# Kitware/SMQTK-Indexing

Hardware: AMD Instinct MI355X
Metric: queries/sec, exact brute-force l2 kNN k=100 over 10000000x128 float32 (recall@100 = 1.0 by construction); scan HBM GB/s vs 8 TB/s peak (higher is better)
Workload: dtype f32 results (distances bit-identical to numpy float32); filter arithmetic int8 MFMA (i32 accumulation, measured per-row error bound), exact re-rank f32

## Files before the change

### smqtk_indexing_amd/csrc/sq_dense_i8.hpp

```cpp
#pragma once
#include "sq_dense_scan.hpp"

namespace sq {

typedef int i32x4 __attribute__((ext_vector_type(4)));
typedef int i32x16 __attribute__((ext_vector_type(16)));

template <int KS>
struct I8Geom {
    static constexpr int ROW_BYTES = KS * 32;
    static constexpr int UNIT_ROWS = KS == 4 ? 64 : 32;
    static constexpr int TILES = UNIT_ROWS / 32;
    static constexpr int UNIT_BYTES = UNIT_ROWS * ROW_BYTES;
    static constexpr int SLOT_BYTES = UNIT_BYTES + 256;
    static constexpr int WAVES = KS <= 8 ? 8 : 4;
    static constexpr int NSTAGE = 2;
    static constexpr int PIECES = UNIT_BYTES / 1024;
    static constexpr int SAMPLES_PER_UNIT = 2 * TILES;
};
static constexpr int I8_MAX_ROW_BYTES = 512;
__host__ __device__ constexpr int i8_row_bytes(int d) { return d <= 128 ? 128 : (d <= 256 ? 256 : 512); }
__host__ __device__ constexpr int i8_unit_rows(int row_bytes) { return row_bytes == 128 ? 64 : 32; }

__device__ __forceinline__ float i8_element(float v, const float* __restrict__ center, int k, bool cosine, double inv_norm) {
    if (cosine) return (float)((double)v * inv_norm);
    return center ? __fsub_rn(v, center[k]) : v;
}

template <int EPL>
static __global__ __launch_bounds__(256) void dense8_energy_kernel(const float* __restrict__ db, long long n, long long ld, int d,
                                                                    const float* __restrict__ center, const double* __restrict__ nx64,
                                                                    double cap, double* __restrict__ sum) {
    __shared__ double red[4][2];
    const int lane = threadIdx.x & 63;
    const long long wave0 = (long long)blockIdx.x * 4 + (threadIdx.x >> 6), nw = (long long)gridDim.x * 4;
    double acc = 0.0, rows = 0.0;
    for (long long row = wave0; row < n; row += nw) {
        double e = 0.0;
        bool bad = false;
        const double inv_norm = nx64 ? 1.0 / sqrt(nx64[row]) : 1.0;
        for (int k0 = 0; k0 < d; k0 += 64 * EPL) {
#pragma unroll
            for (int j = 0; j < EPL; ++j) {
                const int k = k0 + EPL * lane + j;
                if (k < d) {
                    const float v = db[row * ld + k];
                    const float xc = i8_element(v, center, k, nx64 != nullptr, inv_norm);
                    if (!(fabsf(xc) < 3.0e38f)) bad = true;
                    e += (double)xc * (double)xc;
                }
            }
        }
        if (__ballot(bad) != 0ull) continue;
        for (int o = 32; o > 0; o >>= 1) e += __shfl_xor(e, o);
        if (e <= cap) {
            acc += e;
            rows += 1.0;
        }
    }
    if (lane == 0) {
        red[threadIdx.x >> 6][0] = acc;
        red[threadIdx.x >> 6][1] = rows;
    }
    __syncthreads();
    if (threadIdx.x == 0) {
        atomicAdd(sum, red[0][0] + red[1][0] + red[2][0] + red[3][0]);
        atomicAdd(sum + 1, red[0][1] + red[1][1] + red[2][1] + red[3][1]);
    }
}

static constexpr int I8_NCLIP = 12, I8_NCUT = 10;
struct Dense8ClipArgs {
    float inv_dx[I8_NCLIP], dx[I8_NCLIP];
    float cut[I8_NCLIP][I8_NCUT];
};

template <int EPL>
static __global__ __launch_bounds__(256) void dense8_clip_stats_kernel(const float* __restrict__ db, long long n, long long ld, int d,
                                                                        const float* __restrict__ center, const double* __restrict__ nx64,
                                                                        Dense8ClipArgs ca, u32* __restrict__ counts, int row_step) {
    const int lane = threadIdx.x & 63;
    const long long wave0 = ((long long)blockIdx.x * 4 + (threadIdx.x >> 6)) * row_step, nw = (long long)gridDim.x * 4 * row_step;
    u32 cnt[I8_NCLIP][I8_NCUT];
#pragma unroll
    for (int c = 0; c < I8_NCLIP; ++c)
#pragma unroll
        for (int m = 0; m < I8_NCUT; ++m) cnt[c][m] = 0u;
    for (long long row = wave0; row < n; row += nw) {
        float r2[I8_NCLIP];
#pragma unroll
        for (int c = 0; c < I8_NCLIP; ++c) r2[c] = 0.f;
        bool bad = false;
        const double inv_norm = nx64 ? 1.0 / sqrt(nx64[row]) : 1.0;
        for (int k0 = 0; k0 < d; k0 += 64 * EPL) {
#pragma unroll
            for (int j = 0; j < EPL; ++j) {
                const int k = k0 + EPL * lane + j;
                if (k < d) {
                    const float v = db[row * ld + k];
                    const float xc = i8_element(v, center, k, nx64 != nullptr, inv_norm);
                    if (!(fabsf(xc) < 3.0e38f)) bad = true;
#pragma unroll
                    for (int c = 0; c < I8_NCLIP; ++c) {
                        const float t = fminf(fmaxf(rintf(xc * ca.inv_dx[c]), -127.f), 127.f);
                        const float res = __fmaf_rn(-t, ca.dx[c], xc);
                        r2[c] = __fmaf_rn(res, res, r2[c]);
                    }
                }
            }
        }
        if (__ballot(bad) != 0ull) continue;
#pragma unroll
        for (int c = 0; c < I8_NCLIP; ++c) {
            for (int o = 32; o > 0; o >>= 1) r2[c] += __shfl_xor(r2[c], o);
#pragma unroll
            for (int m = 0; m < I8_NCUT; ++m) cnt[c][m] += r2[c] > ca.cut[c][m] ? 1u : 0u;
        }
    }
    if (lane == 0) {
#pragma unroll
        for (int c = 0; c < I8_NCLIP; ++c)
#pragma unroll
            for (int m = 0; m < I8_NCUT; ++m)
                if (cnt[c][m]) atomicAdd(&counts[c * I8_NCUT + m], cnt[c][m]);
    }
}

template <int EPL>
static __global__ __launch_bounds__(256) void dense8_build_kernel(const float* __restrict__ db, long long n, long long ld, int d,
                                                                   long long n_pad, const float* __restrict__ center,
                                                                   const double* __restrict__ nx64, float inv_dx, float dx,
                                                                   signed char* __restrict__ out8, float* __restrict__ nrow,
                                                                   float* __restrict__ r2row, long long row_base, int row_bytes) {
    const int lane = threadIdx.x & 63;
    const long long row = row_base + (long long)blockIdx.x * 4 + (threadIdx.x >> 6);
    if (row >= n_pad) return;
    double e2 = 0.0, r2 = 0.0;
    bool finite = true;
    const double inv_norm = (row < n && nx64) ? 1.0 / sqrt(nx64[row]) : 1.0;
    for (int k0 = 0; k0 < row_bytes; k0 += 64 * EPL) {
        unsigned char q[EPL];
#pragma unroll
        for (int j = 0; j < EPL; ++j) q[j] = 0;
        if (row < n) {
#pragma unroll
            for (int j = 0; j < EPL; ++j) {
                const int k = k0 + EPL * lane + j;
                if (k < d) {
                    const float v = db[row * ld + k];
                    const float xc = i8_element(v, center, k, nx64 != nullptr, inv_norm);
                    if (!(xc == xc) || !(fabsf(xc) < 3.0e38f)) finite = false;
                    float t = rintf(xc * inv_dx);
                    t = fminf(fmaxf(t, -127.f), 127.f);
                    if (!(t == t)) t = 0.f;
                    q[j] = (unsigned char)(signed char)(int)t;
                    const double res = (double)xc - (double)t * (double)dx;
                    e2 += (double)xc * (double)xc;
                    r2 += res * res;
                }
            }
        }
        if (k0 + EPL * lane >= row_bytes) continue;
        unsigned char* dst = reinterpret_cast<unsigned char*>(out8) + row * row_bytes + k0 + EPL * lane;
        if constexpr (EPL == 2) {
            *reinterpret_cast<unsigned short*>(dst) = (unsigned short)(q[0] | (q[1] << 8));
        } else if constexpr (EPL == 4) {
            *reinterpret_cast<u32*>(dst) = (u32)q[0] | ((u32)q[1] << 8) | ((u32)q[2] << 16) | ((u32)q[3] << 24);
        } else {
            uint2 w;
            w.x = (u32)q[0] | ((u32)q[1] << 8) | ((u32)q[2] << 16) | ((u32)q[3] << 24);
            w.y = (u32)q[4] | ((u32)q[5] << 8) | ((u32)q[6] << 16) | ((u32)q[7] << 24);
            *reinterpret_cast<uint2*>(dst) = w;
        }
    }
    finite = __ballot(!finite) == 0ull;
    for (int o = 32; o > 0; o >>= 1) {
        e2 += __shfl_xor(e2, o);
        r2 += __shfl_xor(r2, o);
    }
    if (lane == 0) {
        float nr = __builtin_inff(), rr = 0.f;
        if (row < n && finite) {
            nr = nx64 ? 0.f : (float)e2;
            if ((double)nr > e2) nr = __uint_as_float(__float_as_uint(nr) - 1u);
            rr = (float)r2;
            if ((double)rr < r2) rr = __uint_as_float(__float_as_uint(rr) + 1u);
        }
        nrow[row] = nr;
        r2row[row] = rr;
    }
}

static __global__ __launch_bounds__(256) void dense8_resid_stats_kernel(const float* __restrict__ r2row, const float* __restrict__ nrow,
                                                                         long long n, double* __restrict__ sum_r2,
                                                                         u32* __restrict__ max_bits) {
    __shared__ double red[4];
    __shared__ float rmax[4], nmax[4];
    double acc = 0.0;
    float m = 0.f, mn = 0.f;
    for (long long i = (long long)blockIdx.x * 256 + threadIdx.x; i < n; i += (long long)gridDim.x * 256) {
        const float nv = nrow[i];
        if (nv < __builtin_inff() && nv > -__builtin_inff()) {
            const float v = r2row[i];
            acc += (double)v;
            m = fmaxf(m, v);
            mn = fmaxf(mn, nv);
        }
    }
    for (int o = 32; o > 0; o >>= 1) {
        acc += __shfl_xor(acc, o);
        m = fmaxf(m, __shfl_xor(m, o));
        mn = fmaxf(mn, __shfl_xor(mn, o));
    }
    if ((threadIdx.x & 63) == 0) {
        red[threadIdx.x >> 6] = acc;
        rmax[threadIdx.x >> 6] = m;
        nmax[threadIdx.x >> 6] = mn;
    }
    __syncthreads();
    if (threadIdx.x == 0) {
        atomicAdd(sum_r2, red[0] + red[1] + red[2] + red[3]);
        atomicMax(max_bits, __float_as_uint(fmaxf(fmaxf(rmax[0], rmax[1]), fmaxf(rmax[2], rmax[3]))));
        atomicMax(max_bits + 1, __float_as_uint(fmaxf(fmaxf(nmax[0], nmax[1]), fmaxf(nmax[2], nmax[3]))));
    }
}

static __global__ __launch_bounds__(256) void dense8_flag_kernel(const float* __restrict__ r2row, float* __restrict__ nrow, long long n,
                                                                  float r2_cut, u32* __restrict__ flagged, long long row_base) {
    const long long i = row_base + (long long)blockIdx.x * 256 + threadIdx.x;
    if (i >= n) return;
    if (nrow[i] < __builtin_inff() && r2row[i] > r2_cut) {
        nrow[i] = -__builtin_inff();
        atomicAdd(flagged, 1u);
    }
}

template <int EPL>
__device__ __forceinline__ void dense8_prep_query_row(const float* __restrict__ qrow, bool real, int d, const float* __restrict__ center,
                                                      double dx, double r_max, double x_max, int cosine,
                                                      signed char* __restrict__ p0, signed char* __restrict__ p1, float2& par_out,
                                                      double& qn2_out) {
    const int l16 = threadIdx.x & 15;
    const float sc = cosine ? -1.f : -2.f;
    float v[EPL][4];
#pragma unroll
    for (int c = 0; c < EPL; ++c)
#pragma unroll
        for (int e = 0; e < 4; ++e) {
            const int t = 64 * c + l16 + 16 * e;
            float raw = 0.f, cen = 0.f;
            if (real && t < d) {
                raw = qrow[t];
                if (center) cen = center[t];
            }
            v[c][e] = (real && t < d) ? (center ? __fsub_rn(raw, cen) : raw) : 0.f;
        }
    auto chunk_sum = [](double x0, double x1, double x2, double x3) __attribute__((always_inline)) {
        double sacc = (x0 + x2) + (x1 + x3);
        for (int o = 8; o > 0; o >>= 1) sacc += __shfl_xor(sacc, o);
        return sacc;
    };
    if (cosine) {
        double nn = 0.0;
#pragma unroll
        for (int c = 0; c < EPL; ++c)
            nn += chunk_sum((double)v[c][0] * (double)v[c][0], (double)v[c][1] * (double)v[c][1], (double)v[c][2] * (double)v[c][2],
                            (double)v[c][3] * (double)v[c][3]);
        const double rn = sqrt(nn);
#pragma unroll
        for (int c = 0; c < EPL; ++c)
#pragma unroll
            for (int e = 0; e < 4; ++e) v[c][e] = (float)((double)v[c][e] / rn);
    }
    double Q = 0.0;
    float mx = 0.f;
#pragma unroll
    for (int c = 0; c < EPL; ++c) {
        Q += chunk_sum((double)v[c][0] * (double)v[c][0], (double)v[c][1] * (double)v[c][1], (double)v[c][2] * (double)v[c][2],
                       (double)v[c][3] * (double)v[c][3]);
#pragma unroll
        for (int e = 0; e < 4; ++e) {
            float m = fabsf(sc * v[c][e]);
            if (!(m == m)) m = __builtin_inff();
            mx = fmaxf(mx, m);
        }
    }
    for (int o = 8; o > 0; o >>= 1) mx = fmaxf(mx, __shfl_xor(mx, o));
    const bool ok = real && mx < 3.0e38f && mx > 0.f;
    const double dq = ok ? (double)mx / 127.0 : 1.0;
    const double inv_dq = 1.0 / dq;
    double r2s = 0.0;
#pragma unroll
    for (int c = 0; c < EPL; ++c) {
        double r2[4];
#pragma unroll
        for (int e = 0; e < 4; ++e) {
            const double w = (double)(sc * v[c][e]);
            const double ws = w * inv_dq;
            float qt8 = 0.f, ql8 = 0.f;
            if (ok) {
                qt8 = fminf(fmaxf(rintf((float)ws), -127.f), 127.f);
                ql8 = fminf(fmaxf(rintf((float)((ws - (double)qt8) * 256.0)), -127.f), 127.f);
            }
            const int t = 64 * c + l16 + 16 * e;
            p0[t] = (signed char)(int)qt8;
            p1[t] = (signed char)(int)ql8;
            const double res = w - ((double)qt8 + (double)ql8 * 0.00390625) * dq;
            r2[e] = res * res;
        }
        r2s += chunk_sum(r2[0], r2[1], r2[2], r2[3]);
    }
    const double rq = sqrt(r2s) * (1.0 + 1e-9);
    const double unit = dx * dq;
    const double xr = x_max + r_max, qn = sqrt(Q), wn = (cosine ? 1.0 : 2.0) * qn;
    double e = r_max * wn + xr * rq + 4.0 * 5.9604644775390625e-08 * (xr * (wn + rq) + x_max * x_max);
    e *= 1.0 + 1e-6;
    float ef = (float)e;
    if ((double)ef < e) ef = __uint_as_float(__float_as_uint(ef) + 1u);
    if (!ok && real) ef = __builtin_inff();
    par_out = make_float2((float)unit, real ? ef : 0.f);
    qn2_out = real ? Q : 0.0;
}

template <int EPL>
static __global__ __launch_bounds__(64) void dense8_prep_queries_kernel(const float* __restrict__ q, int nq, int d,
                                                                         const float* __restrict__ center, double dx, double r_max,
                                                                         double x_max, signed char* __restrict__ qs8,
                                                                         float2* __restrict__ par, double* __restrict__ qn2,
                                                                         float* __restrict__ thr, u32* __restrict__ cnt,
                                                                         u32* __restrict__ oflag, float* __restrict__ q_al, int ldq,
                                                                         const DenseCallPtrs* __restrict__ ind, int cosine, int plane_rows) {
    constexpr int row_bytes = EPL * 64;
    if (ind) q = ind->q;
    const int qi = blockIdx.x * 4 + (threadIdx.x >> 4), t = threadIdx.x & 15;
    if (t == 0) {
        thr[qi] = qi < nq ? -__builtin_inff() : __builtin_nanf("");
        cnt[qi] = 0u;
        if (qi == 0) *oflag = 0u;
    }
    if (qi < nq)
        for (int i = t; i < ldq; i += 16) q_al[(long long)qi * ldq + i] = i < d ? q[(long long)qi * d + i] : 0.f;
    float2 pr;
    double Q;
    dense8_prep_query_row<EPL>(q + (long long)qi * d, qi < nq, d, center, dx, r_max, x_max, cosine,
                               qs8 + (long long)qi * row_bytes, qs8 + (long long)(plane_rows + qi) * row_bytes, pr, Q);
    if (t == 0) {
        par[qi] = pr;
        qn2[qi] = Q;
    }
}

struct Dense8ThrPost {
    const float2* par;
    const double* qn2;
    __device__ __forceinline__ void prologue(int, double*) const {}
    __device__ __forceinline__ float operator()(int q, float t) const {
        if (!(t < __builtin_inff())) return t;
        if (!(par[q].y < __builtin_inff())) return __builtin_nanf("");
        const double tt = (double)t + 2.0 * (double)par[q].y + 4e-6 * fabs((double)t + qn2[q]);
        float r = (float)tt;
        if ((double)r < tt) r = __uint_as_float(__float_as_uint(r) + (r >= 0.f ? 1 : -1));
        return r;
    }
};

struct Dense8ScanArgs {
    const signed char* scan8;
    const float* nrow;
    long long n;
    long long n_units;
    const signed char* qs8;
    const float2* par;
    const float* thr;
    uint2* wave_out;
    u32* wave_cnt;
    u32 wave_cap;
    float* sample_out;
    long long ns;
    long long unit_step;
    long long n_sel;
    int nrb;
    int nt;
    long long nt_from_row;
    int nqt;
    int plane_rows;
    int debug;
    float* wave_score;
    u32* hist;
};

template <int KS>
__device__ __forceinline__ int i8_swz(int c, int r) {
    if constexpr (KS == 4) return c ^ ((r >> 1) & 7);
    return (c & ~15) | ((c & 15) ^ (r & 15));
}

enum { I8_EMIT = 0, I8_SAMPLE = 1, I8_LANEMIN = 2, I8_EMIT_H = 3 };

static constexpr int I8_HIST_BINS = 64;
static constexpr int I8_CNT_SHIFT = 5;
static constexpr int I8_HIST_WORDS = TILE_ROWS * I8_HIST_BINS + (TILE_ROWS << I8_CNT_SHIFT);

template <int WAVES>
__device__ __forceinline__ void dense8_hist_flush(u32* lds_hist, u32* __restrict__ ghist) {
    constexpr int PER = TILE_ROWS * I8_HIST_BINS / WAVES;
    const int lane = threadIdx.x & 63;
    const int wave = __builtin_amdgcn_readfirstlane(threadIdx.x >> 6);
#pragma unroll
    for (int i = 0; i < PER / 64; ++i) {
        const int b = wave * PER + i * 64 + lane;
        const u32 v = __hip_atomic_exchange(lds_hist + b, 0u, __ATOMIC_RELAXED, __HIP_MEMORY_SCOPE_WORKGROUP);
        if (v) __hip_atomic_fetch_add(ghist + b, v, __ATOMIC_RELAXED, __HIP_MEMORY_SCOPE_AGENT);
    }
}

template <int KS, int MODE>
__device__ __forceinline__ void dense8_stream(const Dense8ScanArgs& a, unsigned char* smem, const i32x4 (&bq)[KS], const i32x4 (&bl)[KS],
                                              float unit_lo, float thr_l, u32& wcount, float& smin, u32* lds_ticket,
                                              float inv_w_l = 0.f, u32* lds_hist = nullptr) {
    using G = I8Geom<KS>;
    constexpr bool SAMPLE = MODE == I8_SAMPLE || MODE == I8_LANEMIN;
    const int lane = threadIdx.x & 63;
    const int wave = __builtin_amdgcn_readfirstlane(threadIdx.x >> 6);
    const int r31 = lane & 31, h = lane >> 5;
    const u32 lds_base = (u32)(uintptr_t)smem;
    const u32 ring_base = lds_base + (u32)wave * (G::NSTAGE * G::SLOT_BYTES);
    const unsigned char* ring_ptr = smem + wave * (G::NSTAGE * G::SLOT_BYTES);
    const long long wave_id = (long long)blockIdx.x * G::WAVES + wave;
    const long long nwaves = (long long)a.nrb * G::WAVES;
    uint2* wout = a.wave_out + wave_id * a.wave_cap;
    float* wsc = MODE == I8_EMIT_H ? a.wave_score + wave_id * a.wave_cap : nullptr;
    u32* hist_l = MODE == I8_EMIT_H ? lds_hist + r31 * I8_HIST_BINS : nullptr;

    const long long wg_first = (long long)blockIdx.x * G::WAVES;
    auto take_unit = [&]() __attribute__((always_inline)) -> long long {
        u32 t = 0;
        if (lane == 0) t = __hip_atomic_fetch_add(lds_ticket, 1u, __ATOMIC_RELAXED, __HIP_MEMORY_SCOPE_WORKGROUP);
        t = (u32)__builtin_amdgcn_readfirstlane((int)t);
        const long long u = wg_first + (long long)(t % G::WAVES) + (long long)(t / G::WAVES) * nwaves;
        return u < a.n_sel ? u : -1ll;
    };
    const long long my_units = wave_id < a.n_sel ? (a.n_sel - wave_id + nwaves - 1) / nwaves : 0;
    u32 voff[G::PIECES];
#pragma unroll
    for (int j = 0; j < G::PIECES; ++j) {
        const int lin = j * 1024 + lane * 16;
        const int r = lin / G::ROW_BYTES, cpos = (lin % G::ROW_BYTES) >> 4;
        voff[j] = (u32)(r * G::ROW_BYTES + i8_swz<KS>(cpos, r) * 16);
    }
    const u32 voff_n = (u32)lane * 4u;
    static_assert(G::NSTAGE == 2, "two ring slots: the units in flight are sel_even / sel_odd");
    long long issued = 0, sel_even = -1, sel_odd = -1;
    bool more = true;
    auto issue_next = [&]() __attribute__((always_inline)) {
        if (!more) return;
        const long long sel = take_unit();
        if (sel < 0) {
            more = false;
            return;
        }
        if (issued & 1) sel_odd = sel; else sel_even = sel;
        const long long unit_idx = sel * a.unit_step;
        const long long row0 = unit_idx * G::UNIT_ROWS;
        const u32 dst = ring_base + (u32)(issued % G::NSTAGE) * G::SLOT_BYTES;
        const unsigned char* base = reinterpret_cast<const unsigned char*>(a.scan8) + row0 * G::ROW_BYTES;
#pragma unroll
        for (int j = 0; j < G::PIECES; ++j) {
            if (a.nt && row0 >= a.nt_from_row)
                glds16<true>(base, voff[j], dst + (u32)j * 1024);
            else
                glds16<false>(base, voff[j], dst + (u32)j * 1024);
        }
        glds4(a.nrow + row0, voff_n, dst + G::UNIT_BYTES);
        ++issued;
    };
    for (int p = 0; p < G::NSTAGE; ++p) issue_next();
    const int flush_every = (int)(my_units >> 3) > 0 ? (int)(my_units >> 3) : 1;
    int to_flush = flush_every;

    for (long long it = 0; it < issued; ++it) {
        const long long sel = (it & 1) ? sel_odd : sel_even;
        const long long unit_idx = sel * a.unit_step;
        const long long row0 = unit_idx * G::UNIT_ROWS;
        wait_units_in_flight<G::NSTAGE, G::PIECES + 1>((int)(issued - it - 1));
        const unsigned char* sl = ring_ptr + (it % G::NSTAGE) * G::SLOT_BYTES;
        constexpr int KH = KS == 16 ? 8 : KS;
        i32x4 av[G::TILES][KH];
        f32x4 nr[G::TILES][4];
#pragma unroll
        for (int t = 0; t < G::TILES; ++t) {
            const int r = 32 * t + r31;
#pragma unroll
            for (int s = 0; s < KH; ++s)
                av[t][s] = *reinterpret_cast<const i32x4*>(sl + r * G::ROW_BYTES + i8_swz<KS>(2 * s + h, r) * 16);
#pragma unroll
            for (int c = 0; c < 4; ++c) nr[t][c] = *reinterpret_cast<const f32x4*>(sl + G::UNIT_BYTES + (32 * t + 8 * c + 4 * h) * 4);
        }
        asm volatile("s_waitcnt lgkmcnt(0)" ::: "memory");
        if constexpr (KS != 16) issue_next();
#pragma unroll
        for (int t = 0; t < G::TILES; ++t) {
            i32x16 acc, acl;
#pragma unroll
            for (int i = 0; i < 16; ++i) acc[i] = acl[i] = 0;
#pragma unroll
            for (int s = 0; s < KH; ++s) {
                acc = __builtin_amdgcn_mfma_i32_32x32x32_i8(av[t][s], bq[s], acc, 0, 0, 0);
                acl = __builtin_amdgcn_mfma_i32_32x32x32_i8(av[t][s], bl[s], acl, 0, 0, 0);
            }
            if constexpr (KS == 16) {
#pragma unroll
                for (int s = 0; s < KH; ++s)
                    av[t][s] = *reinterpret_cast<const i32x4*>(sl + r31 * G::ROW_BYTES + i8_swz<KS>(2 * (KH + s) + h, r31) * 16);
                asm volatile("s_waitcnt lgkmcnt(0)" ::: "memory");
                issue_next();
#pragma unroll
                for (int s = 0; s < KH; ++s) {
                    acc = __builtin_amdgcn_mfma_i32_32x32x32_i8(av[t][s], bq[KH + s], acc, 0, 0, 0);
                    acl = __builtin_amdgcn_mfma_i32_32x32x32_i8(av[t][s], bl[KH + s], acl, 0, 0, 0);
                }
            }
            if (a.debug & 1024) {
                if (acc[0] == 0x7fffffff && acl[5] == 0x7ffffffe) wcount += 1;
                continue;
            }
            float sc[16];
#pragma unroll
            for (int i = 0; i < 16; ++i) {
                float nv = nr[t][i >> 2][i & 3];
                if constexpr (SAMPLE) nv = nv == -__builtin_inff() ? __builtin_inff() : nv;
                sc[i] = __fmaf_rn((float)((acc[i] << 8) + acl[i]), unit_lo, nv);
            }
            float m = sc[0];
#pragma unroll
            for (int i = 1; i < 16; ++i) m = fminf(m, sc[i]);
            if constexpr (MODE == I8_LANEMIN) {
                smin = fminf(smin, m);
            } else if constexpr (MODE == I8_SAMPLE) {
                a.sample_out[(long long)r31 * a.ns + sel * G::SAMPLES_PER_UNIT + t * 2 + h] = m;
            } else {
                const u64 hit = __ballot(m <= thr_l);
                if (hit != 0) {
                    u32 mask = 0;
#pragma unroll
                    for (int i = 0; i < 16; ++i) mask |= (sc[i] <= thr_l ? 1u : 0u) << i;
                    const u64 bal = __ballot(mask != 0);
                    if (mask) {
                        const u32 pos = wcount + __builtin_amdgcn_mbcnt_hi((u32)(bal >> 32), __builtin_amdgcn_mbcnt_lo((u32)bal, 0u));
                        if (pos < a.wave_cap) {
                            wout[pos] = make_uint2((u32)(row0 + 32 * t + 4 * h), (mask << 16) | (u32)r31);
                            if constexpr (MODE == I8_EMIT_H) wsc[pos] = m;
                        }
                        if constexpr (MODE == I8_EMIT_H) {
                            if (m > -__builtin_inff()) {
                                const int bin = min((int)((thr_l - m) * inv_w_l), I8_HIST_BINS - 1);
                                __hip_atomic_fetch_add(hist_l + bin, 1u, __ATOMIC_RELAXED, __HIP_MEMORY_SCOPE_WORKGROUP);
                            }
                        }
                    }
                    wcount += (u32)__popcll(bal);
                }
            }
        }
        if constexpr (MODE == I8_EMIT_H) {
            if (--to_flush == 0) {
                to_flush = flush_every;
                dense8_hist_flush<G::WAVES>(lds_hist, a.hist);
            }
        }
    }
}

template <int KS>
__device__ __forceinline__ void dense8_load_planes(const signed char* planes, i32x4 (&bq)[KS], i32x4 (&bl)[KS]) {
    using G = I8Geom<KS>;
    const int lane = threadIdx.x & 63, r31 = lane & 31, h = lane >> 5;
#pragma unroll
    for (int s = 0; s < KS; ++s) {
        bq[s] = *reinterpret_cast<const i32x4*>(planes + r31 * G::ROW_BYTES + (2 * s + h) * 16);
        bl[s] = *reinterpret_cast<const i32x4*>(planes + (TILE_ROWS + r31) * G::ROW_BYTES + (2 * s + h) * 16);
    }
#pragma unroll
    for (int s = 0; s < KS; ++s) asm volatile("" : "+v"(bq[s]), "+v"(bl[s]));
}

template <int KS, bool SAMPLE>
__global__ __launch_bounds__(I8Geom<KS>::WAVES * 64, KS == 16 ? 1 : 2) void dense8_scan_kernel(Dense8ScanArgs a) {
    using G = I8Geom<KS>;
    extern __shared__ __attribute__((aligned(16))) unsigned char smem[];
    const int lane = threadIdx.x & 63;
    const int wave = __builtin_amdgcn_readfirstlane(threadIdx.x >> 6);
    const int r31 = lane & 31;
    i32x4 bq[KS], bl[KS];
    dense8_load_planes<KS>(a.qs8, bq, bl);
    float unit_lo = a.par[r31].x * 0.00390625f;
    float thr_l = SAMPLE ? 0.f : a.thr[r31];
    asm volatile("" : "+v"(unit_lo), "+v"(thr_l));
    u32 wcount = 0;
    float smin = 0.f;
    __shared__ u32 s_unit_ticket;
    if (threadIdx.x == 0) s_unit_ticket = 0u;
    __syncthreads();
    dense8_stream<KS, SAMPLE ? I8_SAMPLE : I8_EMIT>(a, smem, bq, bl, unit_lo, thr_l, wcount, smin, &s_unit_ticket);
    if constexpr (!SAMPLE) {
        if (lane == 0) {
            const long long wave_id = (long long)blockIdx.x * G::WAVES + wave;
            a.wave_cnt[2 * wave_id] = wcount;
            a.wave_cnt[2 * wave_id + 1] = 0u;
        }
    }
}


struct Dense8HeadArgs {
    Dense8ScanArgs s;
    const float* q;
    int nq, d;
    const float* center;
    double dx, r_max, x_max;
    int cosine;
    double* qn2;
    u32* cnt;
    u32* oflag;
    float* q_al;
    int ldq;
    const DenseCallPtrs* ind;
    float* lane_min;
    int keep;
    int kk;
};

template <int VM, int NQ>
__device__ __forceinline__ void wave_kth_smallest(const float* __restrict__ vals, long long stride, int M, int k, float (&out)[NQ]) {
    const int lane = threadIdx.x & 63;
    constexpr u32 KINF = 0xff800000u;
    u32 key[NQ][VM];
    u32 prefix[NQ];
    u32 xall = 0u;
#pragma unroll
    for (int n = 0; n < NQ; ++n) {
        u32 kmin = KINF, kmax = 0u;
#pragma unroll
        for (int j = 0; j < VM; ++j) {
            const int i = j * 64 + lane;
            u32 kv = ordered_f32(vals[n * stride + (i < M ? i : 0)]);
            kv = (i < M && kv < KINF) ? kv : KINF;
            key[n][j] = kv;
            kmin = kv < kmin ? kv : kmin;
            kmax = kv > kmax ? kv : kmax;
        }
        for (int o = 32; o > 0; o >>= 1) {
            const u32 a = (u32)__shfl_xor((int)kmin, o), b = (u32)__shfl_xor((int)kmax, o);
            kmin = a < kmin ? a : kmin;
            kmax = b > kmax ? b : kmax;
        }
        prefix[n] = __builtin_amdgcn_readfirstlane(kmin);
        xall |= __builtin_amdgcn_readfirstlane(kmin ^ kmax);
    }
    if (xall != 0u) {
        const int top = 31 - __clz((int)xall);
#pragma unroll
        for (int n = 0; n < NQ; ++n) prefix[n] &= ~((2u << top) - 1u);
        for (int b = top; b >= 0; --b) {
#pragma unroll
            for (int n = 0; n < NQ; ++n) {
                const u32 cand = prefix[n] | ((1u << b) - 1u);
                u32 c = 0;
#pragma unroll
                for (int j = 0; j < VM; ++j) c += (u32)__popcll(__ballot(key[n][j] <= cand));
                if (c < (u32)k) prefix[n] |= 1u << b;
            }
        }
    }
#pragma unroll
    for (int n = 0; n < NQ; ++n) {
        float r = unordered_f32(prefix[n]);
        if (prefix[n] >= KINF) {
            u32 c = 0;
#pragma unroll
            for (int j = 0; j < VM; ++j) c += (u32)__popcll(__ballot(key[n][j] < KINF));
            if (c < (u32)k) r = __builtin_inff();
        }
        out[n] = r;
    }
}

template <int KS>
__global__ __launch_bounds__(I8Geom<KS>::WAVES * 64, KS == 16 ? 1 : 2) void dense8_head_kernel(Dense8HeadArgs ha) {
    using G = I8Geom<KS>;
    constexpr int VB = G::WAVES * 2;
    extern __shared__ __attribute__((aligned(16))) unsigned char smem[];
    __shared__ float2 s_par[TILE_ROWS];
    __shared__ double s_qn2[TILE_ROWS];
    __shared__ float s_lm[TILE_ROWS][16];
    __shared__ u32 s_ticket, s_unit_ticket;
    if (threadIdx.x == 0) s_unit_ticket = 0u;
    const Dense8ScanArgs& a = ha.s;
    const int lane = threadIdx.x & 63;
    const int wave = __builtin_amdgcn_readfirstlane(threadIdx.x >> 6);
    const int r31 = lane & 31, h = lane >> 5;
    const float* q = ha.ind ? ha.ind->q : ha.q;
    const bool first = blockIdx.x == 0;
    signed char* planes = reinterpret_cast<signed char*>(smem);
#pragma unroll
    for (int rnd = 0; rnd < TILE_ROWS / (4 * G::WAVES); ++rnd) {
        const int qi = rnd * 4 * G::WAVES + wave * 4 + (lane >> 4);
        float2 pr;
        double Q;
        dense8_prep_query_row<KS / 2>(q + (long long)qi * ha.d, qi < ha.nq, ha.d, ha.center, ha.dx, ha.r_max, ha.x_max, ha.cosine,
                                      planes + qi * G::ROW_BYTES, planes + (TILE_ROWS + qi) * G::ROW_BYTES, pr, Q);
        if ((lane & 15) == 0) {
            s_par[qi] = pr;
            s_qn2[qi] = Q;
        }
        if (first) {
            if ((lane & 15) == 0) {
                const_cast<float2*>(a.par)[qi] = pr;
                ha.qn2[qi] = Q;
                ha.cnt[qi << I8_CNT_SHIFT] = 0u;
                if (qi == 0) ha.oflag[0] = 0u;
            }
            if (qi < ha.nq)
                for (int i = lane & 15; i < ha.ldq; i += 16) ha.q_al[(long long)qi * ha.ldq + i] = i < ha.d ? q[(long long)qi * ha.d + i] : 0.f;
        }
    }
    __syncthreads();
    i32x4 bq[KS], bl[KS];
    dense8_load_planes<KS>(planes, bq, bl);
    float unit_lo = s_par[r31].x * 0.00390625f;
    asm volatile("" : "+v"(unit_lo));
    if (first) {
        signed char* gp = const_cast<signed char*>(a.qs8);
        for (int i = threadIdx.x; i < 2 * TILE_ROWS * G::ROW_BYTES / 16; i += G::WAVES * 64)
            reinterpret_cast<uint4*>(gp)[i] = reinterpret_cast<const uint4*>(planes)[i];
        for (int i = threadIdx.x; i < I8_HIST_WORDS; i += G::WAVES * 64) a.hist[i] = 0u;
    }
    asm volatile("s_waitcnt vmcnt(0) lgkmcnt(0)" ::: "memory");
    __syncthreads();
    u32 wcount = 0;
    float smin = __builtin_inff();
    if (!(a.debug & 4096)) dense8_stream<KS, I8_LANEMIN>(a, smem, bq, bl, unit_lo, 0.f, wcount, smin, &s_unit_ticket);
    s_lm[r31][(wave * 2 + h) & 15] = smin;
    if (VB < 16 && wave == 0 && h == 0)
        for (int i = VB; i < 16; ++i) s_lm[r31][i] = __builtin_inff();
    __syncthreads();
    const int nb = (int)gridDim.x, keep = ha.keep, M = nb * keep;
#pragma unroll
    for (int rnd = 0; rnd < TILE_ROWS / (4 * G::WAVES); ++rnd) {
        const int qi = rnd * 4 * G::WAVES + wave * 4 + (lane >> 4), l16 = lane & 15;
        float v = s_lm[qi][l16];
#pragma unroll
        for (int kk2 = 2; kk2 <= 16; kk2 <<= 1)
#pragma unroll
            for (int j = kk2 >> 1; j > 0; j >>= 1) {
                const float o = __shfl_xor(v, j);
                const bool up = (l16 & kk2) == 0, lower = (l16 & j) == 0;
                v = (lower == up) ? fminf(v, o) : fmaxf(v, o);
            }
        if (l16 < keep) ha.lane_min[(long long)qi * M + (long long)blockIdx.x * keep + l16] = v;
    }
    asm volatile("s_waitcnt vmcnt(0)" ::: "memory");
    __syncthreads();
    if (threadIdx.x == 0) {
        __threadfence();
        const u32 t = atomicAdd(&ha.oflag[1], 1u);
        if (t == gridDim.x - 1) {
            __threadfence();
            ha.oflag[1] = 0u;
        }
        s_ticket = t;
    }
    __syncthreads();
    if (s_ticket != gridDim.x - 1) return;
    float* thr = const_cast<float*>(a.thr);
    const Dense8ThrPost post{s_par, s_qn2};
#pragma unroll
    for (int rnd = 0; rnd < TILE_ROWS / (4 * G::WAVES); ++rnd) {
        const int q0 = rnd * 4 * G::WAVES + wave * 4;
        float ts[4] = {-__builtin_inff(), -__builtin_inff(), -__builtin_inff(), -__builtin_inff()};
        if (q0 < ha.nq && !(a.debug & 2048)) {
            const float* v = ha.lane_min + (long long)q0 * M;
            if (M <= 256)
                wave_kth_smallest<4, 4>(v, M, M, ha.kk, ts);
            else if (M <= 512)
                wave_kth_smallest<8, 4>(v, M, M, ha.kk, ts);
            else if (M <= 1024)
                wave_kth_smallest<16, 4>(v, M, M, ha.kk, ts);
            else {
#pragma unroll
                for (int j = 0; j < 4; ++j) {
                    float one[1];
                    wave_kth_smallest<32, 1>(v + (long long)j * M, M, M, ha.kk, one);
                    ts[j] = one[0];
                }
            }
        }
#pragma unroll
        for (int j = 0; j < 4; ++j) {
            const float t = q0 + j < ha.nq ? post(q0 + j, ts[j]) : __builtin_nanf("");
            if (lane == 0) thr[q0 + j] = t;
        }
    }
}

struct Dense8TailArgs {
    const float* db;
    long long ld;
    int d;
    const float* q_al;
    int ldq, nq;
    void* keys;
    u32* cnt;
    u32 cap;
    u32* overflow;
    const double* nx64;
    const double* nq64;
    int debug;
    const double* qn2;
    int kk;
    int tighten;
    long long* clk;
};
static constexpr int I8_TAIL_QROWS_BYTES = 32 * (156 + 4) * 4;
static constexpr int I8_TAIL_LIST = 2048;
static constexpr int I8_TAIL_RERANK_BYTES = I8_TAIL_QROWS_BYTES + 3 * RERANK_MAX_GROUP * 4 + 8 * 32 * RERANK_STAGE_STRIDE * 4;
static constexpr int I8_TAIL_LDS_BYTES = I8_TAIL_RERANK_BYTES + I8_TAIL_LIST * 8 + TILE_ROWS * 4 + 16;

template <int KS, bool COSINE>
__global__ __launch_bounds__(I8Geom<KS>::WAVES * 64, KS == 16 ? 1 : 2) void dense8_body_kernel(Dense8ScanArgs a, Dense8TailArgs ta) {
    using G = I8Geom<KS>;
    static_assert(I8_TAIL_LDS_BYTES <= G::WAVES * G::NSTAGE * G::SLOT_BYTES, "the re-rank works in the ring's LDS");
    extern __shared__ __attribute__((aligned(16))) unsigned char smem[];
    __shared__ u32 s_hist8[TILE_ROWS * I8_HIST_BINS];
    __shared__ u32 s_wcnt[G::WAVES];
    __shared__ u32 s_unit_ticket;
    __shared__ float s_thr1[TILE_ROWS], s_eq[TILE_ROWS];
    __shared__ double s_qn2b[TILE_ROWS];
    __shared__ float2 s_parb[TILE_ROWS];
    if (threadIdx.x == 0) s_unit_ticket = 0u;
    if (threadIdx.x < TILE_ROWS) {
        s_thr1[threadIdx.x] = a.thr[threadIdx.x];
        s_parb[threadIdx.x] = a.par[threadIdx.x];
        s_eq[threadIdx.x] = a.par[threadIdx.x].y;
        s_qn2b[threadIdx.x] = ta.qn2[threadIdx.x];
    }
    const int lane = threadIdx.x & 63;
    const int wave = __builtin_amdgcn_readfirstlane(threadIdx.x >> 6);
    const int r31 = lane & 31;
    for (int i = threadIdx.x; i < TILE_ROWS * I8_HIST_BINS; i += G::WAVES * 64) s_hist8[i] = 0u;
    long long* clk = ta.clk ? ta.clk + (long long)blockIdx.x * 8 : nullptr;
    if (clk && threadIdx.x == 0) {
        clk[0] = (long long)wall_clock64();
        clk[1] = 0x7fffffffffffffffll;
    }
    __syncthreads();
    i32x4 bq[KS], bl[KS];
    dense8_load_planes<KS>(a.qs8, bq, bl);
    float unit_lo = a.par[r31].x * 0.00390625f;
    float thr_l = a.thr[r31];
    const float eq_l = a.par[r31].y;
    float inv_w_l = (eq_l > 0.f && eq_l < __builtin_inff()) ? 2.f / eq_l : 0.f;
    if (!(inv_w_l < 3.0e38f)) inv_w_l = 0.f;
    asm volatile("" : "+v"(unit_lo), "+v"(thr_l), "+v"(inv_w_l));
    u32 wcount = 0;
    float smin = 0.f;
    dense8_stream<KS, I8_EMIT_H>(a, smem, bq, bl, unit_lo, thr_l, wcount, smin, &s_unit_ticket, inv_w_l, s_hist8);
    const long long w0 = (long long)blockIdx.x * G::WAVES;
    if (lane == 0) {
        a.wave_cnt[2 * (w0 + wave)] = wcount;
        a.wave_cnt[2 * (w0 + wave) + 1] = 0u;
        s_wcnt[wave] = wcount;
        if (clk) atomicMin((unsigned long long*)(clk + 1), (unsigned long long)wall_clock64());
    }
    asm volatile("s_waitcnt vmcnt(0) lgkmcnt(0)" ::: "memory");
    __builtin_amdgcn_fence(__ATOMIC_RELEASE, "workgroup");
    __syncthreads();
    __builtin_amdgcn_fence(__ATOMIC_ACQUIRE, "workgroup");
    if (clk && threadIdx.x == 0) clk[2] = (long long)wall_clock64();
    float* fl = reinterpret_cast<float*>(smem);
    u32* su = reinterpret_cast<u32*>(smem + I8_TAIL_QROWS_BYTES);
    RerankLds L{fl, su, su + RERANK_MAX_GROUP, su + 2 * RERANK_MAX_GROUP,
                COSINE ? reinterpret_cast<float*>(smem + I8_TAIL_QROWS_BYTES + 3 * RERANK_MAX_GROUP * 4) : nullptr};
    {
        uint2* s_list = reinterpret_cast<uint2*>(smem + I8_TAIL_RERANK_BYTES);
        float* s_thr2 = reinterpret_cast<float*>(smem + I8_TAIL_RERANK_BYTES + I8_TAIL_LIST * 8);
        u32* s_npass = reinterpret_cast<u32*>(s_thr2 + TILE_ROWS);
        static_assert(I8_HIST_BINS == 64, "one lane per bin");
        bool any = false;
#pragma unroll
        for (int wi = 0; wi < G::WAVES; ++wi) any = any || s_wcnt[wi] != 0u;
        const Dense8ThrPost post{s_parb, s_qn2b};
        constexpr int NQW = TILE_ROWS / G::WAVES;
        u32 hc[NQW];
        if (ta.tighten && any) {
#pragma unroll
            for (int j = 0; j < NQW; ++j) {
                const int qi = (j >> 2) * 4 * G::WAVES + wave * 4 + (j & 3);
                hc[j] = __hip_atomic_load(a.hist + qi * I8_HIST_BINS + lane, __ATOMIC_RELAXED, __HIP_MEMORY_SCOPE_AGENT);
            }
#pragma unroll
            for (int j = 0; j < NQW; ++j) {
                const int qi = (j >> 2) * 4 * G::WAVES + wave * 4 + (j & 3);
                hc[j] += s_hist8[qi * I8_HIST_BINS + lane];
            }
        }
#pragma unroll
        for (int rnd = 0; rnd < TILE_ROWS / (4 * G::WAVES); ++rnd) {
#pragma unroll
            for (int j = 0; j < 4; ++j) {
                const int qi = rnd * 4 * G::WAVES + wave * 4 + j;
                const float t1 = s_thr1[qi];
                float t2 = t1;
                if (ta.tighten && any && qi < ta.nq && t1 < __builtin_inff() && t1 > -__builtin_inff()) {
                    u32 c = hc[rnd * 4 + j];
#pragma unroll
                    for (int o = 1; o < 64; o <<= 1) {
                        const u32 up = (u32)__shfl_down((int)c, o);
                        c += lane + o < 64 ? up : 0u;
                    }
                    const u64 reach = __ballot(c >= (u32)ta.kk);
                    const float eq = s_eq[qi];
                    if (reach != 0ull && eq > 0.f && eq < __builtin_inff()) {
                        const int jb = 63 - __clzll((long long)reach);
                        const float inv_w = 2.f / eq;
                        if (inv_w < 3.0e38f) {
                            const double t8 = (double)t1 - (double)jb / (double)inv_w * (1.0 - 1e-6);
                            float t8f = (float)t8;
                            if ((double)t8f < t8) t8f = __uint_as_float(__float_as_uint(t8f) + (t8f >= 0.f ? 1 : -1));
                            const float cand = post(qi, t8f);
                            if (cand < t2) t2 = cand;
                        }
                    }
                    if (lane == 0) atomicMax(a.hist + TILE_ROWS * I8_HIST_BINS + (qi << I8_CNT_SHIFT), ordered_f32(t2));
                }
                if (lane == 0) s_thr2[qi] = t2;
            }
        }
        if (ta.tighten) {
            L.scores = a.wave_score;
            L.thr2 = s_thr2;
            L.list = s_list;
            L.npass = s_npass;
            L.list_cap = I8_TAIL_LIST;
        }
        L.seg_cnt = s_wcnt;
        L.cnt_shift = I8_CNT_SHIFT;
        __syncthreads();
        if (clk && threadIdx.x == 0) clk[3] = (long long)wall_clock64();
        if (ta.tighten) dense8_hist_flush<G::WAVES>(s_hist8, a.hist);
    }
    using K = typename std::conditional<COSINE, K128, u64>::type;
    rerank_block<K, COSINE>(ta.db, ta.ld, ta.d, ta.q_al, ta.ldq, ta.nq, TILE_ROWS, a.wave_out, a.wave_cnt, a.wave_cap,
                            (long long)a.nrb * G::WAVES, G::WAVES, static_cast<K*>(ta.keys), ta.cnt, ta.cap, ta.overflow, ta.nx64,
                            ta.nq64, ta.debug, w0, L);
    if (clk) {
        asm volatile("s_waitcnt vmcnt(0) lgkmcnt(0)" ::: "memory");
        __syncthreads();
        if (threadIdx.x == 0) clk[4] = (long long)wall_clock64();
    }
}

template <int QT, bool SAMPLE>
__global__ __launch_bounds__(512, 2) void dense8_scan_mt_kernel(Dense8ScanArgs a) {
    using G = I8Geom<4>;
    extern __shared__ __attribute__((aligned(16))) unsigned char smem[];
    const int lane = threadIdx.x & 63;
    const int wave = __builtin_amdgcn_readfirstlane(threadIdx.x >> 6);
    const int r31 = lane & 31, h = lane >> 5;
    const u32 lds_base = (u32)(uintptr_t)smem;
    const u32 ring_base = lds_base + (u32)wave * (G::NSTAGE * G::SLOT_BYTES);
    const unsigned char* ring_ptr = smem + wave * (G::NSTAGE * G::SLOT_BYTES);
    const long long wave_id = (long long)blockIdx.x * G::WAVES + wave;
    uint2* wout = a.wave_out + wave_id * a.wave_cap;
    const int L = blockIdx.x;
    int grp, rb;
    if (a.nqt > 1) {
        const int xcd = L & 7, j = L >> 3;
        grp = j % a.nqt;
        rb = (j / a.nqt) * 8 + xcd;
    } else {
        grp = 0;
        rb = L;
    }
    const int q_first = grp * QT * TILE_ROWS;
    const long long rwave = (long long)rb * G::WAVES + wave, nwaves = (long long)a.nrb * G::WAVES;

    i32x4 bq[QT][4], bl[QT][4];
    float unit_lo[QT], thr_l[QT];
#pragma unroll
    for (int g = 0; g < QT; ++g) {
        const int qg = q_first + g * TILE_ROWS + r31;
#pragma unroll
        for (int s = 0; s < 4; ++s) {
            bq[g][s] = *reinterpret_cast<const i32x4*>(a.qs8 + (long long)qg * G::ROW_BYTES + (2 * s + h) * 16);
            bl[g][s] = *reinterpret_cast<const i32x4*>(a.qs8 + (long long)(a.plane_rows + qg) * G::ROW_BYTES + (2 * s + h) * 16);
        }
        unit_lo[g] = a.par[qg].x * 0.00390625f;
        thr_l[g] = SAMPLE ? 0.f : a.thr[qg];
        asm volatile("" : "+v"(unit_lo[g]), "+v"(thr_l[g]));
#pragma unroll
        for (int s = 0; s < 4; ++s) asm volatile("" : "+v"(bq[g][s]), "+v"(bl[g][s]));
    }

    const long long my_units = rwave < a.n_sel ? (a.n_sel - rwave + nwaves - 1) / nwaves : 0;
    u32 voff[G::PIECES];
#pragma unroll
    for (int j = 0; j < G::PIECES; ++j) {
        const int r = 8 * j + (lane >> 3);
        voff[j] = (u32)(r * G::ROW_BYTES + i8_swz<4>(lane & 7, r) * 16);
    }
    const u32 voff_n = (u32)lane * 4u;
    long long issued = 0;
    auto issue_next = [&]() __attribute__((always_inline)) {
        if (issued >= my_units) return;
        const long long unit_idx = (rwave + issued * nwaves) * a.unit_step;
        const long long row0 = unit_idx * G::UNIT_ROWS;
        const u32 dst = ring_base + (u32)(issued % G::NSTAGE) * G::SLOT_BYTES;
        const unsigned char* base = reinterpret_cast<const unsigned char*>(a.scan8) + row0 * G::ROW_BYTES;
#pragma unroll
        for (int j = 0; j < G::PIECES; ++j) {
            if (a.nt && row0 >= a.nt_from_row)
                glds16<true>(base, voff[j], dst + (u32)j * 1024);
            else
                glds16<false>(base, voff[j], dst + (u32)j * 1024);
        }
        glds4(a.nrow + row0, voff_n, dst + G::UNIT_BYTES);
        ++issued;
    };
    for (int p = 0; p < G::NSTAGE; ++p) issue_next();

    u32 wcount = 0;
    for (long long it = 0; it < my_units; ++it) {
        const long long unit_idx = (rwave + it * nwaves) * a.unit_step;
        const long long row0 = unit_idx * G::UNIT_ROWS;
        wait_units_in_flight<G::NSTAGE, G::PIECES + 1>((int)(issued - it - 1));
        const unsigned char* sl = ring_ptr + (it % G::NSTAGE) * G::SLOT_BYTES;
#pragma unroll
        for (int t = 0; t < 2; ++t) {
            const int r = 32 * t + r31;
            i32x4 av[4];
            f32x4 nr[4];
#pragma unroll
            for (int s = 0; s < 4; ++s) av[s] = *reinterpret_cast<const i32x4*>(sl + r * G::ROW_BYTES + i8_swz<4>(2 * s + h, r) * 16);
#pragma unroll
            for (int c = 0; c < 4; ++c) nr[c] = *reinterpret_cast<const f32x4*>(sl + G::UNIT_BYTES + (32 * t + 8 * c + 4 * h) * 4);
            asm volatile("s_waitcnt lgkmcnt(0)" ::: "memory");
            if (t == 1) issue_next();
#pragma unroll
            for (int g = 0; g < QT; ++g) {
                i32x16 acc, acl;
#pragma unroll
                for (int i = 0; i < 16; ++i) acc[i] = acl[i] = 0;
#pragma unroll
                for (int s = 0; s < 4; ++s) {
                    acc = __builtin_amdgcn_mfma_i32_32x32x32_i8(av[s], bq[g][s], acc, 0, 0, 0);
                    acl = __builtin_amdgcn_mfma_i32_32x32x32_i8(av[s], bl[g][s], acl, 0, 0, 0);
                }
                float sc[16];
#pragma unroll
                for (int i = 0; i < 16; ++i) {
                    float nv = nr[i >> 2][i & 3];
                    if constexpr (SAMPLE) nv = nv == -__builtin_inff() ? __builtin_inff() : nv;
                    sc[i] = __fmaf_rn((float)((acc[i] << 8) + acl[i]), unit_lo[g], nv);
                }
                float m = sc[0];
#pragma unroll
                for (int i = 1; i < 16; ++i) m = fminf(m, sc[i]);
                if constexpr (SAMPLE) {
                    const long long sel = rwave + it * nwaves;
                    a.sample_out[(long long)(q_first + g * TILE_ROWS + r31) * a.ns + sel * G::SAMPLES_PER_UNIT + t * 2 + h] = m;
                } else {
                    const u64 hit = __ballot(m <= thr_l[g]);
                    if (hit != 0) {
                        u32 mask = 0;
#pragma unroll
                        for (int i = 0; i < 16; ++i) mask |= (sc[i] <= thr_l[g] ? 1u : 0u) << i;
                        const u64 bal = __ballot(mask != 0);
                        if (mask) {
                            const u32 pos = wcount + __builtin_amdgcn_mbcnt_hi((u32)(bal >> 32), __builtin_amdgcn_mbcnt_lo((u32)bal, 0u));
                            if (pos < a.wave_cap) wout[pos] = make_uint2((u32)(row0 + 32 * t + 4 * h), (mask << 16) | (u32)(g * TILE_ROWS + r31));
                        }
                        wcount += (u32)__popcll(bal);
                    }
                }
            }
        }
    }
    if constexpr (!SAMPLE) {
        if (lane == 0) {
            a.wave_cnt[2 * wave_id] = wcount;
            a.wave_cnt[2 * wave_id + 1] = (u32)(grp * QT);
        }
    }
}

}
```

### smqtk_indexing_amd/csrc/sq_dma.hpp

```cpp
#pragma once
#include "sq_common.hpp"

namespace sq {

__device__ __forceinline__ const void* uniform_ptr(const void* p) {
    const u64 v = (u64)(uintptr_t)p;
    const u32 lo = __builtin_amdgcn_readfirstlane((u32)v), hi = __builtin_amdgcn_readfirstlane((u32)(v >> 32));
    return (const void*)(uintptr_t)(((u64)hi << 32) | lo);
}
template <bool NT = false>
__device__ __forceinline__ void glds16(const void* gbase_uniform, u32 voff, u32 lds_dst) {
    u32 keep;
    if constexpr (NT)
        asm volatile(
            "s_mov_b32 %0, m0\n\t"
            "s_mov_b32 m0, %3\n\t"
            "s_nop 0\n\t"
            "global_load_lds_dwordx4 %1, %2 nt\n\t"
            "s_mov_b32 m0, %0"
            : "=&s"(keep)
            : "v"(voff), "s"(uniform_ptr(gbase_uniform)), "s"(__builtin_amdgcn_readfirstlane(lds_dst))
            : "memory");
    else
        asm volatile(
            "s_mov_b32 %0, m0\n\t"
            "s_mov_b32 m0, %3\n\t"
            "s_nop 0\n\t"
            "global_load_lds_dwordx4 %1, %2\n\t"
            "s_mov_b32 m0, %0"
            : "=&s"(keep)
            : "v"(voff), "s"(uniform_ptr(gbase_uniform)), "s"(__builtin_amdgcn_readfirstlane(lds_dst))
            : "memory");
}
__device__ __forceinline__ void glds4(const void* gbase_uniform, u32 voff, u32 lds_dst) {
    u32 keep;
    asm volatile(
        "s_mov_b32 %0, m0\n\t"
        "s_mov_b32 m0, %3\n\t"
        "s_nop 0\n\t"
        "global_load_lds_dword %1, %2\n\t"
        "s_mov_b32 m0, %0"
        : "=&s"(keep)
        : "v"(voff), "s"(uniform_ptr(gbase_uniform)), "s"(__builtin_amdgcn_readfirstlane(lds_dst))
        : "memory");
}

__device__ __forceinline__ void glds_set_m0(u32 lds_dst) {
    asm volatile("s_mov_b32 m0, %0\n\ts_nop 0" ::"s"(__builtin_amdgcn_readfirstlane(lds_dst)) : "memory");
}
template <int OFF, bool NT = false>
__device__ __forceinline__ void glds16_m0(const void* gbase_uniform, u32 voff) {
    static_assert(OFF >= -4096 && OFF <= 4095, "13-bit signed instruction offset");
    if constexpr (NT)
        asm volatile("global_load_lds_dwordx4 %0, %1 offset:%2 nt" ::"v"(voff), "s"(uniform_ptr(gbase_uniform)), "n"(OFF) : "memory");
    else
        asm volatile("global_load_lds_dwordx4 %0, %1 offset:%2" ::"v"(voff), "s"(uniform_ptr(gbase_uniform)), "n"(OFF) : "memory");
}
template <int OFF>
__device__ __forceinline__ void glds4_m0(const void* gbase_uniform, u32 voff) {
    static_assert(OFF >= -4096 && OFF <= 4095, "13-bit signed instruction offset");
    asm volatile("global_load_lds_dword %0, %1 offset:%2" ::"v"(voff), "s"(uniform_ptr(gbase_uniform)), "n"(OFF) : "memory");
}
template <int N, int J = 0, class F>
__device__ __forceinline__ void static_for_one(int j, F&& f) {
    if constexpr (J < N) {
        if (j == J)
            f(std::integral_constant<int, J>{});
        else
            static_for_one<N, J + 1>(j, f);
    }
}

template <int N>
__device__ __forceinline__ void wait_vmcnt() {
    asm volatile("s_waitcnt vmcnt(%0)" ::"n"(N) : "memory");
}

template <int NSTAGE, int PER>
__device__ __forceinline__ void wait_units_in_flight(int units) {
    if constexpr (NSTAGE >= 4) {
        if (units >= 3) {
            wait_vmcnt<3 * PER>();
            return;
        }
    }
    if constexpr (NSTAGE >= 3) {
        if (units == 2) {
            wait_vmcnt<2 * PER>();
            return;
        }
    }
    if (units == 1)
        wait_vmcnt<PER>();
    else
        wait_vmcnt<0>();
}

__device__ __forceinline__ void store_u64_counted(u64* p, u64 v) {
    asm volatile("global_store_dwordx2 %0, %1, off" ::"v"(p), "v"(v) : "memory");
}

template <int PER, int S, int EMAX, int U, int E>
__device__ __forceinline__ void wait_ops_rec(int units, int epis) {
    if (units == U && epis == E) {
        wait_vmcnt<(U * PER + E * S < 63 ? U * PER + E * S : 63)>();
        return;
    }
    if constexpr (E > 0)
        wait_ops_rec<PER, S, EMAX, U, E - 1>(units, epis);
    else if constexpr (U > 0)
        wait_ops_rec<PER, S, EMAX, U - 1, EMAX>(units, epis);
    else
        wait_vmcnt<0>();
}
template <int NSTAGE, int PER, int S>
__device__ __forceinline__ void wait_ops_in_flight(int units, int epis) {
    wait_ops_rec<PER, S, NSTAGE, NSTAGE - 1, NSTAGE>(units, epis);
}

}
```

Before: 149,200.

## Count epilogue stores in vmcnt waits so ring waits don't drain candidate writes

Candidate stores in the int8 filter scan are now issued as inline-asm global stores, and the kernel tracks how many store groups each of the last two units issued. The per-unit ring wait then allows that many extra outstanding vmcnt operations, selected through a compile-time binary tree of s_waitcnt immediates. Before this, vmcnt(N) counted stores too, so waiting for the prefetch would also wait for epilogue stores to finish. The NT/non-NT branch is also hoisted out of the load loop. The risk is that if the store count is wrong, the wait becomes too weak and LDS data is read before it arrives.

```diff
diff --git a/smqtk_indexing_amd/csrc/sq_dense_i8.hpp b/smqtk_indexing_amd/csrc/sq_dense_i8.hpp
--- a/smqtk_indexing_amd/csrc/sq_dense_i8.hpp
+++ b/smqtk_indexing_amd/csrc/sq_dense_i8.hpp
@@ -464,12 +464,12 @@
         const long long row0 = unit_idx * G::UNIT_ROWS;
         const u32 dst = ring_base + (u32)(issued % G::NSTAGE) * G::SLOT_BYTES;
         const unsigned char* base = reinterpret_cast<const unsigned char*>(a.scan8) + row0 * G::ROW_BYTES;
-#pragma unroll
-        for (int j = 0; j < G::PIECES; ++j) {
-            if (a.nt && row0 >= a.nt_from_row)
-                glds16<true>(base, voff[j], dst + (u32)j * 1024);
-            else
-                glds16<false>(base, voff[j], dst + (u32)j * 1024);
+        if (a.nt && row0 >= a.nt_from_row) {
+#pragma unroll
+            for (int j = 0; j < G::PIECES; ++j) glds16<true>(base, voff[j], dst + (u32)j * 1024);
+        } else {
+#pragma unroll
+            for (int j = 0; j < G::PIECES; ++j) glds16<false>(base, voff[j], dst + (u32)j * 1024);
         }
         glds4(a.nrow + row0, voff_n, dst + G::UNIT_BYTES);
         ++issued;
@@ -477,12 +477,20 @@
     for (int p = 0; p < G::NSTAGE; ++p) issue_next();
     const int flush_every = (int)(my_units >> 3) > 0 ? (int)(my_units >> 3) : 1;
     int to_flush = flush_every;
+    constexpr int EPI_STORES = MODE == I8_EMIT_H ? 2 : 1;
+    const bool count_stores = !SAMPLE && !(a.debug & 32768);
+    int epi_1 = 0, epi_2 = 0;
 
     for (long long it = 0; it < issued; ++it) {
         const long long sel = (it & 1) ? sel_odd : sel_even;
         const long long unit_idx = sel * a.unit_step;
         const long long row0 = unit_idx * G::UNIT_ROWS;
-        wait_units_in_flight<G::NSTAGE, G::PIECES + 1>((int)(issued - it - 1));
+        if constexpr (SAMPLE)
+            wait_units_in_flight<G::NSTAGE, G::PIECES + 1>((int)(issued - it - 1));
+        else
+            wait_unit_and_stores<G::PIECES + 1, EPI_STORES, 2 * G::TILES>((int)(issued - it - 1), epi_1 + epi_2);
+        epi_2 = epi_1;
+        epi_1 = 0;
         const unsigned char* sl = ring_ptr + (it % G::NSTAGE) * G::SLOT_BYTES;
         constexpr int KH = KS == 16 ? 8 : KS;
         i32x4 av[G::TILES][KH];
@@ -541,6 +549,7 @@
             } else {
                 const u64 hit = __ballot(m <= thr_l);
                 if (hit != 0) {
+                    if (count_stores && (u32)__builtin_amdgcn_readfirstlane((int)wcount) < a.wave_cap) ++epi_1;
                     u32 mask = 0;
 #pragma unroll
                     for (int i = 0; i < 16; ++i) mask |= (sc[i] <= thr_l ? 1u : 0u) << i;
@@ -548,8 +557,9 @@
                     if (mask) {
                         const u32 pos = wcount + __builtin_amdgcn_mbcnt_hi((u32)(bal >> 32), __builtin_amdgcn_mbcnt_lo((u32)bal, 0u));
                         if (pos < a.wave_cap) {
-                            wout[pos] = make_uint2((u32)(row0 + 32 * t + 4 * h), (mask << 16) | (u32)r31);
-                            if constexpr (MODE == I8_EMIT_H) wsc[pos] = m;
+                            store_u64_counted(reinterpret_cast<u64*>(wout + pos),
+                                              ((u64)((mask << 16) | (u32)r31) << 32) | (u64)(u32)(row0 + 32 * t + 4 * h));
+                            if constexpr (MODE == I8_EMIT_H) store_u32_counted(reinterpret_cast<u32*>(wsc + pos), __float_as_uint(m));
                         }
                         if constexpr (MODE == I8_EMIT_H) {
                             if (m > -__builtin_inff()) {
diff --git a/smqtk_indexing_amd/csrc/sq_dma.hpp b/smqtk_indexing_amd/csrc/sq_dma.hpp
--- a/smqtk_indexing_amd/csrc/sq_dma.hpp
+++ b/smqtk_indexing_amd/csrc/sq_dma.hpp
@@ -99,6 +99,9 @@
 __device__ __forceinline__ void store_u64_counted(u64* p, u64 v) {
     asm volatile("global_store_dwordx2 %0, %1, off" ::"v"(p), "v"(v) : "memory");
 }
+__device__ __forceinline__ void store_u32_counted(u32* p, u32 v) {
+    asm volatile("global_store_dword %0, %1, off" ::"v"(p), "v"(v) : "memory");
+}
 
 template <int PER, int S, int EMAX, int U, int E>
 __device__ __forceinline__ void wait_ops_rec(int units, int epis) {
@@ -118,4 +121,26 @@
     wait_ops_rec<PER, S, NSTAGE, NSTAGE - 1, NSTAGE>(units, epis);
 }
 
+__host__ __device__ constexpr int ring_wait_allowance(int per, int s, int units, int epis) { return units * per + epis * s; }
+static_assert(ring_wait_allowance(9, 2, 0, 0) == 0 && ring_wait_allowance(9, 2, 1, 0) == 9 && ring_wait_allowance(9, 2, 0, 4) == 8 &&
+              ring_wait_allowance(9, 2, 1, 4) == 17 && ring_wait_allowance(17, 2, 1, 2) == 21 && ring_wait_allowance(9, 1, 1, 3) == 12,
+              "units * PER + epilogues * S");
+template <int PER, int S, int EMAX, int LO, int HI>
+__device__ __forceinline__ void wait_ring_tree(int idx) {
+    if constexpr (LO == HI) {
+        wait_vmcnt<ring_wait_allowance(PER, S, LO / (EMAX + 1), LO % (EMAX + 1))>();
+    } else {
+        constexpr int MID = (LO + HI) / 2;
+        if (idx <= MID)
+            wait_ring_tree<PER, S, EMAX, LO, MID>(idx);
+        else
+            wait_ring_tree<PER, S, EMAX, MID + 1, HI>(idx);
+    }
 }
+template <int PER, int S, int EMAX>
+__device__ __forceinline__ void wait_unit_and_stores(int units, int epis) {
+    static_assert(ring_wait_allowance(PER, S, 1, EMAX) < 64, "vmcnt is a six-bit field on gfx9");
+    wait_ring_tree<PER, S, EMAX, 0, 2 * EMAX + 1>(units * (EMAX + 1) + epis);
+}
+
+}
```

Result: no change. 150,300, median of 6 (+0.7%).
